# Genie-Kim/PintheMemory

Measured on AMD Instinct MI355X. Metric: train imgs/sec 768x768 bs=8 R50-DeepLabV3+ +mem, higher is better.
Workload: dtype f32

## Files before the change

### include/pinmem_hip.h

```cpp
#ifndef PINMEM_HIP_H
#define PINMEM_HIP_H
#include <stddef.h>
#include <stdint.h>

#ifdef __cplusplus
extern "C" {
#endif

typedef enum pm_status { PM_OK = 0, PM_EINVAL = -1, PM_EWORKSPACE = -2, PM_ELAUNCH = -3, PM_EUNSUPPORTED = -4 } pm_status;

typedef enum pm_dtype { PM_F32 = 0, PM_BF16 = 1 } pm_dtype;
#define PM_TF_ZERO_PAD64 1

typedef struct pm_tensor {
  void* ptr;
  int32_t n, h, w, c;
  int64_t pitch;
  int32_t dtype;
  int32_t flags;
} pm_tensor;

#define PM_ABI_VERSION 420

typedef struct pm_conv_params {
  int32_t struct_size;
  int32_t kh, kw, stride, pad, dil;
  int32_t prec;
  void* wino_v;
  int64_t wino_v_bytes;
  void* wxf;
  int64_t wxf_bytes;
  int32_t wxf_valid;
} pm_conv_params;

typedef struct pm_conv_epilogue {
  int64_t struct_size;
  const float* bias;
  const float* scale;
  const float* shift;
  const float* residual;
  int64_t residual_pitch;
  int32_t relu;
  float* bn_partials;
  int64_t bn_partials_bytes;
} pm_conv_epilogue;

const char* pm_last_error(void);
int pm_version(void);

size_t pm_conv_workspace(const pm_tensor* x, const pm_tensor* y, const pm_conv_params* p, int which );
size_t pm_conv_winograd_v_bytes(const pm_tensor* x, const pm_tensor* y, const pm_conv_params* p);
size_t pm_conv_wxf_bytes(const pm_tensor* x, const pm_tensor* y, const pm_conv_params* p);
size_t pm_conv_wxf_bytes_dgrad(const pm_tensor* dy, const pm_tensor* dx, const pm_conv_params* p);
typedef struct pm_wxf_job {
  const float* w;
  void* wxf;
  int64_t wxf_bytes;
  int32_t cout, kh, kw, cin;
  int32_t dgrad;
  int32_t reserved;
} pm_wxf_job;
int pm_conv_wxf_refresh_bf16(const pm_wxf_job* jobs, int n, void* stream);
int pm_conv_wxf_refresh_f32(const pm_wxf_job* jobs, int n, void* stream);
size_t pm_conv_bn_partials_bytes(const pm_tensor* x, const pm_tensor* y, const pm_conv_params* p);
int pm_conv_fwd(const pm_tensor* x, const float* w_krsc, const pm_tensor* y, const pm_conv_params* p,
                const pm_conv_epilogue* ep, void* ws, size_t ws_bytes, void* stream);
int pm_conv_bwd_data(const pm_tensor* dy, const float* w_krsc, const pm_tensor* dx, const pm_conv_params* p,
                     const pm_tensor* add, void* ws, size_t ws_bytes, void* stream);
int pm_conv_bwd_data_masked(const pm_tensor* dy, const float* w_krsc, const pm_tensor* dx, const pm_conv_params* p,
                            const pm_tensor* add, const uint8_t* add_mask, void* ws, size_t ws_bytes, void* stream);
int pm_conv_bwd_weight(const pm_tensor* x, const pm_tensor* dy, float* dw_krsc, float* dbias, const pm_conv_params* p,
                       void* ws, size_t ws_bytes, void* stream);

typedef struct pm_routing {
  int32_t struct_size;
  int32_t winograd;
  int32_t winograd_fused;
  int32_t conv16;
  int32_t conv16_wide;
  int32_t conv16_persistent;
  int32_t wgrad16;
  int32_t bf16_wgrad;
  int32_t split;
} pm_routing;
int pm_routing_get(pm_routing* out);
int pm_routing_set(const pm_routing* r);


int pm_set_winograd(int mode);
int pm_set_winograd_fused(int on);
int pm_set_conv16(int on);
int pm_set_bf16_wgrad(int on);
int pm_set_wgrad16(int on);
int pm_set_split(int on);

int pm_profile_enable(int on);
int pm_profile_dump(const char* csv_path);
int pm_profile_read(int mode, int bm, int bn, int km, int nst, double* total_ms, double* total_flops, int64_t* launches, int clear);
int pm_profile_read_prec(int mode, int bm, int bn, int km, int nst, int prec, double* total_ms, double* total_flops, int64_t* launches, int clear);
int pm_profile_read_bytes(int mode, int bm, int bn, int km, int nst, int prec, double* total_bytes);

size_t pm_bn_workspace(const pm_tensor* x);
int pm_bn_stats(const pm_tensor* x, float* moments, void* ws, size_t ws_bytes, void* stream);
int pm_bn_stats_finalize(const pm_tensor* x, float eps, float* mean, float* invstd, float* running_mean , float* running_var ,
                         float momentum, void* ws, size_t ws_bytes, void* stream);
int pm_bn_merge(const float* parts, int world, int c, float* moments, void* stream);
// ... 162 lines not shown
```

### pinthememory_amd/build.py

```python
import os
import subprocess
import sys

HERE = os.path.dirname(os.path.abspath(__file__))
CSRC = os.path.join(HERE, 'csrc')
LIB = os.path.join(HERE, 'libpinmem_hip.so')
SOURCES = ['misc.hip', 'bf16.hip', 'conv_igemm.hip', 'conv_split.hip', 'pwstream.hip', 'conv16.hip', 'conv16w.hip', 'wgrad16.hip', 'winograd.hip', 'bn.hip', 'pool_resize.hip', 'loss.hip', 'memory.hip', 'augment.hip', 'resample.hip']
FLAGS = ['--offload-arch=gfx950', '-O3', '-std=c++17', '-fPIC', '-ffp-contract=fast', '-Wall', '-Wno-unused-function']


STAMP = LIB + '.stamp'


def _fingerprint():
    import hashlib
    h = hashlib.sha256(' '.join(FLAGS).encode())
    for path in sorted(os.path.join(CSRC, f) for f in os.listdir(CSRC)) + [os.path.join(HERE, '..', 'include', 'pinmem_hip.h')]:
        h.update(os.path.basename(path).encode())
        with open(path, 'rb') as f:
            h.update(f.read())
    return h.hexdigest()


def _stale():
    if not (os.path.exists(LIB) and os.path.exists(STAMP)):
        return True
    with open(STAMP) as f:
        return f.read().strip() != _fingerprint()


# ... 47 lines not shown
```

### pinthememory_amd/csrc/conv_igemm.hip

```cpp
#include <stdlib.h>
#include <algorithm>
#include <type_traits>
#include <vector>

#include "pm_common.h"

#include "conv_igemm_kernel.h"

namespace {

template <int ZL, bool O16 = false>
__global__ __launch_bounds__(256) void splitk_reduce_vec_kernel(const float* __restrict__ ws, int ksplit, long slab, int M, int Nn,
                                                                float* __restrict__ C, long c_pitch, const float* bias,
                                                                const float* scale, const float* shift, const float* residual,
                                                                long res_pitch, int relu, const unsigned char* res_mask) {
  constexpr int GP = 256 / ZL;
  __shared__ float4 red[ZL > 1 ? ZL : 1][GP];
  const int gl = threadIdx.x % GP, zl = threadIdx.x / GP;
  const long groups = (long)M * Nn / 4;
  for (long g0 = (long)blockIdx.x * GP; g0 < groups; g0 += (long)gridDim.x * GP) {
    const long grp = g0 + gl;
    float4 v = make_float4(0.f, 0.f, 0.f, 0.f);
    if (grp < groups)
#pragma unroll 8
// ... 281 lines not shown
    if (k.prec == 2) return launch_prec<MODE, BM, BN, WM, WN, KM, 2>(k, grid, smem, st);
  }
  if constexpr (MODE == MODE_WGRAD && BN >= 64) {
    if (k.prec == 3) return launch_prec<MODE, BM, BN, WM, WN, KM, 3>(k, grid, smem, st);
    if (k.prec == 4) return launch_prec<MODE, BM, BN, WM, WN, KM, 4>(k, grid, smem, st);
  }
  if (k.prec != 0) launch_prec<MODE, BM, BN, WM, WN, KM, 1>(k, grid, smem, st);
  else launch_prec<MODE, BM, BN, WM, WN, KM, 0>(k, grid, smem, st);
}
template <int MODE, int BM, int BN, int WM, int WN>
void launch_one(const ConvK& k, dim3 grid, size_t smem, hipStream_t st) {
  if (k.kmode == K_SMALL) launch_inst<MODE, BM, BN, WM, WN, K_SMALL>(k, grid, smem, st);
  else if (k.kmode == K_FAST && MODE != MODE_WGRAD) launch_inst<MODE, BM, BN, WM, WN, (MODE != MODE_WGRAD ? K_FAST : K_MID)>(k, grid, smem, st);
  else launch_inst<MODE, BM, BN, WM, WN, K_MID>(k, grid, smem, st);
}

struct ProfRec {
  hipEvent_t a, b;
  int mode, bm, bn, km, prec, nst;
  int M, Nn, K, batch, ksplit;
  double flops;
  double bytes;
};
bool g_prof_on = false;
std::vector<ProfRec> g_prof;
struct ProfScope {
  ProfRec rec{};
  hipStream_t st;
  ProfScope(hipStream_t st_, int mode, int bm, int bn, int km, int prec, int nst, long M, long Nn, long K, int batch, int ksplit, double flops, double bytes = 0.0) : st(st_) {
    if (!g_prof_on) return;
    (void)hipEventCreate(&rec.a), (void)hipEventCreate(&rec.b);
    rec.mode = mode, rec.bm = bm, rec.bn = bn, rec.km = km, rec.prec = prec, rec.nst = nst, rec.M = (int)M, rec.Nn = (int)Nn, rec.K = (int)K, rec.batch = batch, rec.ksplit = ksplit;
    rec.flops = flops, rec.bytes = bytes;
    (void)hipEventRecord(rec.a, st);
  }
  void done() {
    if (!g_prof_on) return;
    (void)hipEventRecord(rec.b, st);
    g_prof.push_back(rec);
  }
};

template <class K>
void set_epilogue(K& k, const pm_conv_epilogue& e) {
  k.bias = e.bias, k.scale = e.scale, k.shift = e.shift, k.residual = e.residual, k.res_pitch = e.residual_pitch, k.relu = e.relu;
}
// ... 20 lines not shown
    k.batch_xcd = units >= 8 && (rem == 0 || ((rem == 1 || rem == 2 || rem == 4) && ntile % (8 / rem) == 0));
  }
  const int km = (MODE == MODE_WGRAD && k.kmode == K_FAST) ? K_MID : ((k.prec == 5 && MODE != MODE_WGRAD && k.kmode == K_FAST && k.kh * k.kw == 1 && k.stride == 1 && k.pad == 0 && !k.sub) ? K_PW : k.kmode);
  ProfScope prof(st, MODE, p.bm, p.bn, km, k.prec, lds_stages(MODE, k.kmode, p.bn, k.kper), k.M, k.Nn, k.K, batch, p.ksplit,
                 flops >= 0.0 ? flops : 2.0 * (double)k.M * (double)k.Nn * (double)k.K * batch,
                 (double)batch * ((double)k.a_bytes + (double)k.b_bytes + ((k.io16 && p.ksplit == 1) ? 2.0 : 4.0) * (double)k.M * (double)k.Nn * (double)p.ksplit));
  if constexpr (MODE != MODE_WGRAD) {
    if (pm_route.split && (k.prec == 0 || k.prec == 5) && !k.io16 && batch == 1 && p.ksplit == 1 && !k.stats && k.kh * k.kw == 1 && k.stride == 1 && k.pad == 0 && !k.sub) {
      pm_gemm_pw g;
      g.A = k.A, g.B = k.B, g.C = k.C, g.res_mask = k.res_mask;
      set_epilogue(g, pm_conv_epilogue{(int64_t)sizeof(pm_conv_epilogue), k.bias, k.scale, k.shift, k.residual, k.res_pitch, k.relu, nullptr, 0});
      g.a_pitch = MODE == MODE_FWD ? k.x_pitch : k.y_pitch, g.c_pitch = k.c_pitch;
      g.b_sn = MODE == MODE_FWD ? k.K : 1, g.b_sk = MODE == MODE_FWD ? 1 : k.Nn;
      g.M = k.M, g.Nn = k.Nn, g.K = k.K;
      if (pm_pwstream_ok(&g)) {
        prof.rec.bm = 32, prof.rec.bn = 64, prof.rec.km = 4, prof.rec.prec = 5, prof.rec.nst = 0;
        const int e = pm_pwstream_launch(&g, st);
        prof.done();
        return e;
      }
    }
  }
  constexpr bool akc = MODE != MODE_WGRAD, bkc = MODE == MODE_FWD;
  if (k.prec == 5) {
    if (int e = pm_conv_split_launch(MODE, p.bm, p.bn, k, grid.x, grid.y, grid.z, pm_conv_split_stage_bytes(MODE, p.bm, p.bn), st)) return e;
    prof.rec.nst = 1;
    prof.done();
    return pm_check_launch("conv_split");
  }
  const bool tr = MODE == MODE_WGRAD && (k.prec == 3 || k.prec == 4) && p.bn >= 64;
  auto smem = [&](int bm, int bn) {
    if (tr) return (size_t)2 * ((k.prec == 4 ? 2 : 1) * BK * (bm + 32) + (k.prec == 4 ? 2 : 1) * BK * (bn + 32)) * 2;
    return (size_t)2 * ((akc ? bm * LDK : BK * bm) + (bkc ? bn * LDK : BK * bn)) * sizeof(float);
  };
  if (p.bm == 64) {
    if (p.bn == 128) launch_one<MODE, 64, 128, 2, 2>(k, grid, smem(64, 128), st);
    else launch_one<MODE, 64, 64, 2, 2>(k, grid, smem(64, 64), st);
  } else if (p.bn == 128) {
    launch_one<MODE, 128, 128, 2, 2>(k, grid, smem(128, 128), st);
  } else if (p.bn == 64) {
    launch_one<MODE, 128, 64, 2, 2>(k, grid, smem(128, 64), st);
  } else {
    launch_one<MODE, 128, 32, 4, 1>(k, grid, smem(128, 32), st);
  }
  prof.done();
  return pm_check_launch("conv_igemm");
// ... 25 lines not shown
  }
  PM_REQUIRE(x->c % 4 == 0, PM_EUNSUPPORTED, "conv: Cin %% 4 != 0 unsupported (pad the input channels)");
  PM_REQUIRE((y->c % 4 == 0) || (p->kh * p->kw == 1), PM_EUNSUPPORTED, "conv: Cout %% 4 != 0 only for 1x1");
  PM_REQUIRE(x->pitch >= x->c && y->pitch >= y->c, PM_EINVAL, "conv: pitch < channels");
  PM_REQUIRE(pm_pixels(x) * x->pitch < (1ll << 29) && pm_pixels(y) * y->pitch < (1ll << 29) && (int64_t)y->c * x->c * p->kh * p->kw < (1ll << 29),
             PM_EUNSUPPORTED, "conv: tensor too large for 32-bit byte offsets (2 GiB per tensor)");
  return PM_OK;
}

void fill_geom(ConvK& k, const pm_tensor* x, const pm_tensor* y, const pm_conv_params* p) {
  k.N = x->n, k.H = x->h, k.W = x->w, k.Cin = x->c, k.x_pitch = x->pitch;
  k.Ho = y->h, k.Wo = y->w, k.Cout = y->c, k.y_pitch = y->pitch;
  k.kh = p->kh, k.kw = p->kw, k.stride = p->stride, k.pad = p->pad, k.dil = p->dil;
  k.sshift = p->stride == 2 ? 1 : 0;
  k.prec = p->prec != 0 ? 1 : 0;
  k.T_eff = p->kh * p->kw, k.tk_w = p->kw, k.ky0 = k.kx0 = 0, k.ksy = k.ksx = 1;
  k.sub = k.sub_cy = k.sub_cx = 0, k.Hc = x->h, k.Wc = x->w;
  k.bias = k.scale = k.shift = k.residual = nullptr;
  k.res_pitch = 0, k.res_mask = nullptr, k.relu = 0, k.stats = nullptr, k.io16 = 0;
  k.stage_ep = 1;
  k.spl_prio = 1;
  k.n_group = 8;
  k.batch_xcd = 0;
  k.a_bs = k.b_bs = k.c_bs = 0;
}

struct WinoPlan {
  bool use;
  pm_wino_geom g;
  int Kp, P;
  size_t v_bytes, m_bytes, u_bytes;
  Plan pl;
};
inline bool wino_wgrad_pays(int cin, int cout) { return (long)cin * cout >= 256 * 256; }
WinoPlan wino_plan(const pm_tensor* xin, int cout, const pm_conv_params* p, bool wgrad = false) {
  WinoPlan wp{};
  if (wgrad && !wino_wgrad_pays(xin->c, cout)) return wp;
  if (pm_route.winograd == 0 || p->kh != 3 || p->kw != 3 || p->stride != 1 || p->pad != p->dil || p->prec != 0) return wp;
  const int cin = xin->c;
  if (cin < 128 || cout < 128 || (cout & 3) || (cin & 3)) return wp;
  int m = 0;
  double best_ratio = 0.6;
  for (int cand = pm_route.winograd; cand >= 2; cand -= 2) {
    const pm_wino_geom g = pm_wino_make_geom(xin->n, xin->h, xin->w, p->dil, cand);
    const double cover = (double)(cand * g.TY * p->dil) * (double)(cand * g.TX * p->dil) / ((double)xin->h * xin->w);
    const double ratio = cover * (cand + 2) * (cand + 2) / (9.0 * cand * cand);
// ... 354 lines not shown
}

enum RouteKind {
  R_DIRECT,
  R_WINO,
  R_BF16,
  R_S2_NATIVE,
  R_S2_PARITY,
  R_WINO_WGRAD,
  R_BF16_WGRAD,
  R_DIRECT_WGRAD,
};
struct ConvRoute {
  RouteKind kind;
  Plan pl;
  WinoPlan wino;
  WinoWgradPlan wino_w;
  Bf16Plan b16;
  pm_conv_params pe;
  S2Native s2n;
  S2ParityPlan s2p;
  Bf16WgradPlan b16w;
  W16Plan w16;
  bool native16;
  size_t ws_bytes;
  size_t class_off, slab_off;
  size_t bias_off;
  size_t x32_off, dy32_off;
  size_t v_keep_bytes;
  size_t wxf_bytes;
  size_t bn_bytes;
};

ConvRoute route_conv(int which, const pm_tensor* x, const pm_tensor* y, const pm_conv_params* p) {
  ConvRoute r{};
  long M, Nn, K;
  gemm_dims(which, x, y, p, M, Nn, K);
  if (which == MODE_FWD) {
    if ((r.wino = wino_plan(x, y->c, p)).use) {
      r.kind = R_WINO, r.ws_bytes = wino_ws(r.wino), r.wxf_bytes = r.wino.u_bytes;
      r.v_keep_bytes = wino_wgrad_pays(x->c, y->c) ? r.wino.v_bytes : 0;
    } else if (p->prec == 2 && (r.b16 = bf16_plan(x, y, p)).use) {
      r.kind = R_BF16, r.pe = *p, r.ws_bytes = bf16_ws(r.b16), r.wxf_bytes = r.b16.wb_bytes;
    } else {
      r.kind = R_DIRECT, r.pl = make_plan(MODE_FWD, M, Nn, K, p->prec != 0), r.ws_bytes = pm_align_up(r.pl.ws_bytes, 256);
    }
    bool bn;
    if (pm_is_bf16(y)) bn = pm_vec8(y) && r.kind == R_BF16 && (r.b16.c16 ? (r.b16.k16.ksplit == 1 && !r.b16.k16.wide) : r.b16.pl.ksplit == 1);
    else if (pm_is_bf16(x) || (y->c & 3) || (y->pitch & 3) || !pm_aligned16(y->ptr)) bn = false;
    else bn = r.kind == R_BF16 ? r.b16.pl.ksplit == 1 : (r.kind == R_DIRECT && p->prec == 0 && r.pl.ksplit == 1 && r.pl.bn >= 64);
    r.bn_bytes = bn ? pm_align_up((size_t)pm_cdiv(pm_pixels(y), 32) * y->c * 2 * sizeof(float), 256) : 0;
  } else if (which == MODE_DGRAD) {
    if (p->stride == 2) {
      if ((r.s2n = s2_native_plan(y, x, p)).ok) {
        r.kind = R_S2_NATIVE, r.ws_bytes = r.s2n.total;
      } else {
        r.kind = R_S2_PARITY, r.s2p = s2_parity_plan(y, x, p);
        r.class_off = 0, r.slab_off = 4 * r.s2p.tmp_bytes;
        r.dy32_off = pm_align_up(r.slab_off + r.s2p.slab_bytes + 256, 256);
        r.ws_bytes = r.dy32_off + upcast_bytes(y);
      }
    } else if (dgrad_bf16_ok(p) && (r.pe = dgrad_as_fwd(p), r.b16 = bf16_plan(y, x, &r.pe)).use) {
      r.kind = R_BF16, r.ws_bytes = bf16_ws(r.b16), r.wxf_bytes = r.b16.wb_bytes;
    } else if ((r.wino = wino_plan(y, x->c, p)).use) {
      r.kind = R_WINO, r.ws_bytes = wino_ws(r.wino);
    } else {
      r.kind = R_DIRECT, r.pl = make_plan(MODE_DGRAD, M, Nn, K, p->prec != 0), r.ws_bytes = pm_align_up(r.pl.ws_bytes, 256);
    }
// ... 28 lines not shown
  const pm_tensor* dy = &dy32;
  float* tmp = (float*)((char*)ws + r.class_off);
  float* slab = (float*)((char*)ws + r.slab_off);
  for (int cls = 0; cls < 4; ++cls) {
    if (!r.s2p.valid[cls]) continue;
    const S2Class& c = r.s2p.c[cls];
    const Plan& pl = r.s2p.pl[cls];
    ConvK k;
    fill_geom(k, dx, dy, p);
    k.A = (const float*)dy->ptr, k.B = w;
    k.M = (int)c.M, k.Nn = dx->c, k.K = c.nky * c.nkx * dy->c;
    k.a_bytes = (unsigned)(pm_pixels(dy) * dy->pitch * 4), k.b_bytes = (unsigned)((long)dy->c * p->kh * p->kw * dx->c * 4);
    k.kmode = dy->c >= BK ? K_MID : K_SMALL;
    k.T_eff = c.nky * c.nkx, k.tk_w = c.nkx, k.ky0 = c.ky0, k.kx0 = c.kx0, k.ksy = c.ksy, k.ksx = c.ksx;
    k.sub = 1, k.sub_cy = c.cy, k.sub_cx = c.cx, k.Hc = c.Hc, k.Wc = c.Wc;
    float* out = (float*)((char*)tmp + cls * r.s2p.tmp_bytes);
    if (int e = run_gemm<MODE_DGRAD>(k, pl, slab, out, (long)dx->c, NO_EPILOGUE, st)) return e;
  }
  return s2_interleave(tmp, (long)(r.s2p.tmp_bytes / sizeof(float)), r.s2p.valid, dx, add, st, "dgrad_s2_interleave");
}

template <int MODE>
int conv_direct(const pm_tensor* x, const pm_tensor* y, const float* w, const pm_conv_params* p, const Plan& pl, const pm_conv_epilogue& e, void* ws, hipStream_t st,
                const unsigned char* res_mask = nullptr) {
  const pm_tensor *xin = MODE == MODE_FWD ? x : y, *out = MODE == MODE_FWD ? y : x;
  long M, Nn, K;
  gemm_dims(MODE, x, y, p, M, Nn, K);
  ConvK k;
  fill_geom(k, x, y, p);
  k.io16 = pm_is_bf16(out) ? 1 : 0;
  k.A = (const float*)xin->ptr, k.B = w;
  k.M = (int)M, k.Nn = (int)Nn, k.K = (int)K;
  k.a_bytes = (unsigned)(pm_pixels(xin) * xin->pitch * 4), k.b_bytes = (unsigned)((long)y->c * p->kh * p->kw * x->c * 4);
  k.kmode = (xin->c % BK == 0 && (MODE == MODE_FWD || p->stride == 1)) ? 0 : (xin->c >= BK ? 1 : 2);
  return run_gemm<MODE>(k, pl, (float*)ws, (float*)out->ptr, (long)out->pitch, e, st, -1.0, res_mask);
}

int conv_wgrad_direct(const pm_tensor* x, const pm_tensor* dy, float* dw, const pm_conv_params* p, const ConvRoute& r, void* ws, hipStream_t st) {
  long M, Nn, K;
  gemm_dims(MODE_WGRAD, x, dy, p, M, Nn, K);
  if (r.w16.use) {
    pm_wgrad16 w16 = r.w16.k;
    ProfScope prof(st, MODE_WGRAD, w16.bm, w16.bn, 2, 4, 3, M, Nn, K, 1, w16.ksplit, 2.0 * (double)M * (double)Nn * (double)K);
    return run_planned(w16.ksplit, M, Nn, (float*)ws, dw, Nn, NO_EPILOGUE, false, nullptr, st, [&](float* C, bool) {
      w16.C = C;
      const int e = pm_wgrad16_launch(&w16, st);
      prof.done();
      return e;
    });
  }
  ConvK k;
  fill_geom(k, x, dy, p);
  if (p->prec == 2) k.prec = 3;
  if (r.native16) {
    PM_REQUIRE(x->c % 8 == 0 && dy->c % 8 == 0 && r.pl.bn >= 64, PM_EUNSUPPORTED, "conv_bwd_weight(bf16): channels %% 8 != 0 or a tile narrower than 64");
    k.prec = 4;
  }
  const int esz = r.native16 ? 2 : 4;
  k.A = (const float*)dy->ptr, k.B = (const float*)x->ptr;
  k.M = (int)M, k.Nn = (int)Nn, k.K = (int)K;
  k.a_bytes = (unsigned)(pm_pixels(dy) * dy->pitch * esz), k.b_bytes = (unsigned)(pm_pixels(x) * x->pitch * esz), k.kmode = dy->w >= (r.native16 ? 2 * BK : BK) ? 1 : 2;
  return run_gemm<MODE_WGRAD>(k, r.pl, (float*)ws, dw, Nn, NO_EPILOGUE, st);
}

}

static pm_routing routing_from_env() {
  auto env = [](const char* name, int dflt) { const char* e = getenv(name); return e ? atoi(e) : dflt; };
  return pm_routing{
      (int32_t)sizeof(pm_routing),
      4,
      env("PM_WINO_FUSED", 0),
      env("PM_CONV16", 1),
      env("PM_C16W", 1),
      env("PM_C16P", 1),
      env("PM_WGRAD16", 1),
      0,
      env("PM_SPLIT", 1),
  };
}
const pm_routing pm_route_defaults = routing_from_env();
pm_routing pm_route = pm_route_defaults;
extern "C" int pm_routing_get(pm_routing* out) {
  PM_REQUIRE(out && out->struct_size == (int32_t)sizeof(pm_routing), PM_EINVAL, "pm_routing_get: struct_size %d != %zu (library ABI %d)", out ? out->struct_size : -1,
             sizeof(pm_routing), PM_ABI_VERSION);
  *out = pm_route;
  return PM_OK;
}
extern "C" int pm_routing_set(const pm_routing* r) {
  PM_REQUIRE(r && r->struct_size == (int32_t)sizeof(pm_routing), PM_EINVAL, "pm_routing_set: struct_size %d != %zu (library ABI %d)", r ? r->struct_size : -1, sizeof(pm_routing),
             PM_ABI_VERSION);
  PM_REQUIRE(r->winograd == 0 || r->winograd == 2 || r->winograd == 4, PM_EINVAL, "pm_routing_set: winograd %d (0, 2 or 4)", r->winograd);
  PM_REQUIRE(r->conv16 >= 0 && r->conv16 <= 2 && r->conv16_wide >= 0 && r->conv16_wide <= 3, PM_EINVAL, "pm_routing_set: conv16 %d / conv16_wide %d", r->conv16, r->conv16_wide);
  pm_route = *r;
  return PM_OK;
}
extern "C" int pm_set_winograd(int mode) {
  PM_REQUIRE(mode == 0 || mode == 2 || mode == 4, PM_EINVAL, "pm_set_winograd: mode %d (0 off, 2 F(2x2,3x3), 4 prefer F(4x4,3x3))", mode);
  pm_route.winograd = mode;
  return PM_OK;
}
extern "C" int pm_set_conv16(int on) {
  PM_REQUIRE(on >= 0 && on <= 8, PM_EINVAL, "pm_set_conv16: %d (0 register-staged, 1 per shape, 2 LDS-DMA everywhere / narrow tiles only, 3 LDS-DMA everywhere / wide tiles "
             "wherever the shape allows, 4 per shape without the wide kernel, 5 / 6 = 1 (the streaming 1x1 kernel left the library in round 6), 7 as 3 with the 256 x 256 tile, "
             "8 as 3 with one block per tile instead of the persistent ring)", on);
  pm_route.conv16 = (on == 3 || on == 7 || on == 8) ? 2 : ((on == 4 || on == 5 || on == 6) ? 1 : on);
  pm_route.conv16_wide = (on == 3 || on == 8) ? 2 : (on == 7 ? 3 : ((on == 2 || on == 4) ? 0 : pm_route_defaults.conv16_wide));
  pm_route.conv16_persistent = on == 8 ? 0 : (on == 3 ? 1 : pm_route_defaults.conv16_persistent);
  return PM_OK;
}
extern "C" int pm_set_winograd_fused(int on) {
  pm_route.winograd_fused = on != 0;
  return PM_OK;
}
extern "C" int pm_set_wgrad16(int on) {
  pm_route.wgrad16 = on != 0;
// ... 60 lines not shown
  }
  fclose(f);
  return PM_OK;
}

extern "C" size_t pm_conv_workspace(const pm_tensor* x, const pm_tensor* y, const pm_conv_params* p0, int which) {
  const pm_conv_params tp = tier_params(p0, x, y);
  return route_conv(which, x, y, &tp).ws_bytes;
}
extern "C" size_t pm_conv_winograd_v_bytes(const pm_tensor* x, const pm_tensor* y, const pm_conv_params* p0) {
  if (!x || !y || !p0) return 0;
  const pm_conv_params tp = tier_params(p0, x, y);
  return route_conv(MODE_FWD, x, y, &tp).v_keep_bytes;
}
extern "C" size_t pm_conv_wxf_bytes(const pm_tensor* x, const pm_tensor* y, const pm_conv_params* p0) {
  if (!x || !y || !p0) return 0;
  const pm_conv_params tp = tier_params(p0, x, y);
  return route_conv(MODE_FWD, x, y, &tp).wxf_bytes;
}
extern "C" size_t pm_conv_wxf_bytes_dgrad(const pm_tensor* dy, const pm_tensor* dx, const pm_conv_params* p0) {
  if (!dy || !dx || !p0) return 0;
  const pm_conv_params tp = tier_params(p0, dy, dx);
  return route_conv(MODE_DGRAD, dx, dy, &tp).wxf_bytes;
}
extern "C" size_t pm_conv_bn_partials_bytes(const pm_tensor* x, const pm_tensor* y, const pm_conv_params* p0) {
  if (!x || !y || !p0 || check_common(x, y, p0) != PM_OK) return 0;
  const pm_conv_params tp = tier_params(p0, x, y);
  return route_conv(MODE_FWD, x, y, &tp).bn_bytes;
}

extern "C" int pm_conv_wxf_refresh_f32(const pm_wxf_job* jobs, int n, void* stream) {
  PM_REQUIRE(n >= 0 && (jobs || n == 0), PM_EINVAL, "conv_wxf_refresh_f32: bad job table");
  std::vector<const float*> w(n);
  std::vector<float*> U(n);
  std::vector<int> cout(n), cin(n), kp(n), m(n);
  for (int i = 0; i < n; ++i) {
    const pm_wxf_job& q = jobs[i];
    PM_REQUIRE(q.w && q.wxf && q.cout > 0 && q.cin > 0 && q.kh == 3 && q.kw == 3 && q.dgrad == 0, PM_EINVAL,
               "conv_wxf_refresh_f32: job %d: forward transforms of 3x3 filters only", i);
    PM_REQUIRE(pm_aligned16(q.wxf), PM_EINVAL, "conv_wxf_refresh_f32: job %d: buffer must be 16-byte aligned", i);
    const int Kp = (q.cin + BK - 1) / BK * BK;
    const size_t u4 = pm_align_up((size_t)36 * q.cout * Kp * sizeof(float), 256), u2 = pm_align_up((size_t)16 * q.cout * Kp * sizeof(float), 256);
    PM_REQUIRE((size_t)q.wxf_bytes == u4 || (size_t)q.wxf_bytes == u2, PM_EINVAL, "conv_wxf_refresh_f32: job %d: %ld bytes is neither the F(4x4) nor the F(2x2) transform of %d x %d",
               i, (long)q.wxf_bytes, q.cout, q.cin);
    w[i] = q.w, U[i] = (float*)q.wxf, cout[i] = q.cout, cin[i] = q.cin, kp[i] = Kp, m[i] = (size_t)q.wxf_bytes == u4 ? 4 : 2;
  }
// ... 11 lines not shown
  PM_REQUIRE(w && pm_aligned16(w), PM_EINVAL, "conv_fwd: weight null or unaligned");
  pm_conv_epilogue e0 = {(int64_t)sizeof(pm_conv_epilogue), nullptr, nullptr, nullptr, nullptr, 0, 0};
  if (ep) e0 = *ep;
  PM_REQUIRE((e0.scale == nullptr) == (e0.shift == nullptr), PM_EINVAL, "conv_fwd: scale and shift go together");
  const ConvRoute r = route_conv(MODE_FWD, x, y, p);
  if (e0.bn_partials) {
    PM_REQUIRE(!e0.relu && !e0.residual, PM_EINVAL, "conv_fwd: bn_partials are the statistics of the convolution output (no residual / ReLU)");
    PM_REQUIRE(r.bn_bytes != 0 && (size_t)e0.bn_partials_bytes >= r.bn_bytes, PM_EINVAL, "conv_fwd: this call cannot emit bn_partials (ask pm_conv_bn_partials_bytes): %zu needed", r.bn_bytes);
  }
  PM_REQUIRE(ws_bytes >= r.ws_bytes && (ws || r.ws_bytes == 0), PM_EWORKSPACE, "conv_fwd: workspace %zu < %zu", ws_bytes, r.ws_bytes);
  hipStream_t st = (hipStream_t)stream;
  switch (r.kind) {
    case R_WINO: {
      float* keep = (p->wino_v && (size_t)p->wino_v_bytes >= r.wino.v_bytes) ? (float*)p->wino_v : nullptr;
      float* uext = (p->wxf && (size_t)p->wxf_bytes >= r.wino.u_bytes) ? (float*)p->wxf : nullptr;
      return wino_conv(x, w, y->c, x->c, false, y, r.wino, e0, ws, st, keep, uext, p->wxf_valid != 0);
    }
    case R_BF16: {
      char* wext = (p->wxf && (size_t)p->wxf_bytes >= r.b16.wb_bytes) ? (char*)p->wxf : nullptr;
      return conv_bf16(x, w, y->c, x->c, false, y, &r.pe, r.b16, e0, ws, st, wext, p->wxf_valid != 0);
    }
    default:
      PM_REQUIRE(pm_is_f32(x), PM_EUNSUPPORTED, "conv_fwd: a bf16 input needs at least 32 channels (got %d)", x->c);
      return conv_direct<MODE_FWD>(x, y, w, p, r.pl, e0, ws, st);
  }
}

extern "C" int pm_conv_bwd_data(const pm_tensor* dy, const float* w, const pm_tensor* dx, const pm_conv_params* p0, const pm_tensor* add,
                                void* ws, size_t ws_bytes, void* stream) {
  return pm_conv_bwd_data_masked(dy, w, dx, p0, add, nullptr, ws, ws_bytes, stream);
}

extern "C" int pm_conv_bwd_data_masked(const pm_tensor* dy, const float* w, const pm_tensor* dx, const pm_conv_params* p0, const pm_tensor* add,
                                       const uint8_t* add_mask, void* ws, size_t ws_bytes, void* stream) {
  if (int e = check_common(dx, dy, p0)) return e;
  const pm_conv_params tp = tier_params(p0, dy, dx);
  const pm_conv_params* p = &tp;
  PM_REQUIRE(!add || (add->ptr && pm_same_shape(add, dx) && add->dtype == dx->dtype), PM_EINVAL, "conv_bwd_data: `add` must match dx (shape and dtype)");
  PM_REQUIRE(!add || !pm_is_bf16(add) || pm_vec8(add), PM_EINVAL, "conv_bwd_data: bf16 `add` must be 16B aligned with pitch %% 8 == 0");
  PM_REQUIRE(w && pm_aligned16(w), PM_EINVAL, "conv_bwd_data: weight null or unaligned");
  const ConvRoute r = route_conv(MODE_DGRAD, dx, dy, p);
  PM_REQUIRE(ws_bytes >= r.ws_bytes && (ws || r.ws_bytes == 0), PM_EWORKSPACE, "conv_bwd_data: workspace %zu < %zu", ws_bytes, r.ws_bytes);
  if (add_mask) {
    PM_REQUIRE(add && pm_is_f32(add) && pm_is_f32(dy) && pm_vec4(add) && pm_vec4(dx), PM_EINVAL, "conv_bwd_data: a masked `add` is an fp32 tensor with 16-byte rows and c %% 4 == 0");
    PM_REQUIRE(r.kind == R_DIRECT, PM_EUNSUPPORTED,
               "conv_bwd_data: a masked `add` is served by the fp32 implicit-GEMM route only (this call routes to %s)",
               r.kind == R_WINO ? "Winograd" : (r.kind == R_BF16 ? "the bf16 kernels" : "the stride-2 class kernels"));
// ... 55 lines not shown
```

### pinthememory_amd/csrc/conv_igemm_parts.h

```cpp
#pragma once
#include <stdint.h>
#include <type_traits>

#include "pm_common.h"

typedef float f32x16 __attribute__((ext_vector_type(16)));
typedef __bf16 bf16x8 __attribute__((ext_vector_type(8)));

struct ConvK {
  const float* A;
  const float* B;
  float* C;
  int N, H, W, Cin;
  int Ho, Wo, Cout;
  long x_pitch, y_pitch;
  int kh, kw, stride, pad, dil, sshift;
  int M, Nn, K;
  int ksplit;
  int kper;
  long c_pitch;
  long c_split;
  long a_bs, b_bs, c_bs;
  int tiles_m, tiles_n;
  unsigned a_bytes, b_bytes;
  int kmode;
  int prec;
  int T_eff, tk_w, ky0, kx0, ksy, ksx;
  int sub, sub_cy, sub_cx, Hc, Wc;
  const float* bias;
  const float* scale;
  const float* shift;
  const float* residual;
  long res_pitch;
  const unsigned char* res_mask;
  int relu;
  float* stats;
  int io16;
  int stage_ep;
  int n_group;
  int batch_xcd;
  int spl_prio;
};

namespace {

enum { MODE_FWD = 0, MODE_DGRAD = 1, MODE_WGRAD = 2 };
constexpr int BK = 32;
constexpr int LDK = 36;
constexpr int LD5 = 52;

typedef float v4f __attribute__((ext_vector_type(4)));
constexpr int OOB = 0x7fffffff;

__device__ __forceinline__ v4f bload(__amdgpu_buffer_rsrc_t r, unsigned off) {
  return __builtin_bit_cast(v4f, __builtin_amdgcn_raw_buffer_load_b128(r, (int)off, 0, 0));
}

__device__ __forceinline__ uint2 pack4(const v4f& v) {
  typedef __bf16 bf16x4 __attribute__((ext_vector_type(4)));
  bf16x4 o;
  o[0] = (__bf16)v.x, o[1] = (__bf16)v.y, o[2] = (__bf16)v.z, o[3] = (__bf16)v.w;
  return __builtin_bit_cast(uint2, o);
}
__device__ __forceinline__ void split4(const v4f& v, uint2& hi, uint2& mid, uint2& lo) {
  const unsigned u0 = __float_as_uint(v.x), u1 = __float_as_uint(v.y), u2 = __float_as_uint(v.z), u3 = __float_as_uint(v.w);
// ... 228 lines not shown
```

### pinthememory_amd/hip/lib.py

```python
import ctypes
import os
from ctypes import POINTER, byref, c_char_p, c_float, c_int, c_int32, c_int64, c_size_t, c_void_p

import torch

_HERE = os.path.dirname(os.path.dirname(os.path.abspath(__file__)))
LIB_PATH = os.environ.get('PM_LIB') or os.path.join(_HERE, 'libpinmem_hip.so')


class PmTensor(ctypes.Structure):
    _fields_ = [('ptr', c_void_p), ('n', c_int32), ('h', c_int32), ('w', c_int32), ('c', c_int32), ('pitch', c_int64), ('dtype', c_int32), ('flags', c_int32)]


PM_F32, PM_BF16 = 0, 1
PM_TF_ZERO_PAD64 = 1


class PmSgdEntry(ctypes.Structure):
    _fields_ = [('param', c_void_p), ('grad', c_void_p), ('momentum_buffer', c_void_p), ('numel', c_int64)]


class PmWxfJob(ctypes.Structure):
    _fields_ = [('w', c_void_p), ('wxf', c_void_p), ('wxf_bytes', c_int64), ('cout', c_int32), ('kh', c_int32), ('kw', c_int32), ('cin', c_int32),
                ('dgrad', c_int32), ('reserved', c_int32)]


class PmConvParams(ctypes.Structure):
    _fields_ = [('struct_size', c_int32), ('kh', c_int32), ('kw', c_int32), ('stride', c_int32), ('pad', c_int32), ('dil', c_int32), ('prec', c_int32),
                ('wino_v', c_void_p), ('wino_v_bytes', c_int64),
                ('wxf', c_void_p), ('wxf_bytes', c_int64), ('wxf_valid', c_int32)]


class PmRouting(ctypes.Structure):
    _fields_ = [('struct_size', c_int32), ('winograd', c_int32), ('winograd_fused', c_int32), ('conv16', c_int32), ('conv16_wide', c_int32),
                ('conv16_persistent', c_int32), ('wgrad16', c_int32), ('bf16_wgrad', c_int32), ('split', c_int32)]


class PmAugImage(ctypes.Structure):
    _fields_ = [('order', ctypes.c_uint8 * 4), ('enabled', ctypes.c_uint8), ('flip', ctypes.c_uint8), ('hue_shift', ctypes.c_uint8), ('reserved', ctypes.c_uint8),
                ('brightness', c_float), ('contrast', c_float), ('saturation', c_float), ('radius', c_int32), ('w', ctypes.c_double * 6)]


class PmGeoImage(ctypes.Structure):
    _fields_ = [('h_in', c_int32), ('w_in', c_int32), ('h', c_int32), ('w', c_int32), ('pad_h', c_int32), ('pad_w', c_int32), ('y1', c_int32), ('x1', c_int32)]


RESAMPLE_MAX_TAPS = 24
RESAMPLE_REC = RESAMPLE_MAX_TAPS + 2


class PmConvEpilogue(ctypes.Structure):
    _fields_ = [('struct_size', c_int64), ('bias', c_void_p), ('scale', c_void_p), ('shift', c_void_p), ('residual', c_void_p),
                ('residual_pitch', c_int64), ('relu', c_int32), ('bn_partials', c_void_p), ('bn_partials_bytes', c_int64)]


def conv_params(kh, kw, stride, pad, dil, prec=0):
    return PmConvParams(ctypes.sizeof(PmConvParams), kh, kw, stride, pad, dil, prec)


def conv_epilogue(*fields):
    return PmConvEpilogue(ctypes.sizeof(PmConvEpilogue), *fields)


ABI_VERSION = 420


class PinmemError(RuntimeError):
    pass


_T, _P, _E = POINTER(PmTensor), POINTER(PmConvParams), POINTER(PmConvEpilogue)
_vp, _sz, _i, _f, _i64 = c_void_p, c_size_t, c_int, c_float, c_int64

SIGNATURES = {
    'pm_last_error': (c_char_p, []),
    'pm_version': (c_int, []),
    'pm_conv_winograd_v_bytes': (_sz, [_T, _T, _P]),
    'pm_conv_wxf_bytes': (_sz, [_T, _T, _P]),
    'pm_conv_wxf_bytes_dgrad': (_sz, [_T, _T, _P]),
    'pm_conv_wxf_refresh_bf16': (_i, [_vp, _i, _vp]),
    'pm_conv_wxf_refresh_f32': (_i, [_vp, _i, _vp]),
    'pm_conv_workspace': (_sz, [_T, _T, _P, _i]),
    'pm_conv_fwd': (_i, [_T, _vp, _T, _P, _E, _vp, _sz, _vp]),
    'pm_conv_bwd_data': (_i, [_T, _vp, _T, _P, _T, _vp, _sz, _vp]),
    'pm_conv_bwd_data_masked': (_i, [_T, _vp, _T, _P, _T, _vp, _vp, _sz, _vp]),
    'pm_conv_bwd_weight': (_i, [_T, _T, _vp, _vp, _P, _vp, _sz, _vp]),
    'pm_set_winograd': (_i, [_i]),
# ... 65 lines not shown
    'pm_label_class_weights_workspace': (_sz, [_i]),
    'pm_label_class_weights': (_i, [_vp, _i, _i, _i, _i, ctypes.c_double, _i, _i, _vp, _vp, _sz, _vp]),
    'pm_upsample_eval_workspace': (_sz, [_T, _i, _i]),
    'pm_upsample_eval': (_i, [_T, _f, _vp, _i, _i, _vp, _vp, _i, _vp, _vp, _sz, _vp]),
    'pm_mem_read_fwd': (_i, [_T, _vp, _i, _vp, _T, _vp, _vp, _vp]),
    'pm_mem_read_fwd_pq_workspace': (_sz, [_i64, _i]),
    'pm_mem_read_fwd_pq': (_i, [_T, _vp, _i, _vp, _vp, _T, _vp, _vp, _vp, _vp, _sz, _vp]),
    'pm_mem_colsoftmax_workspace': (_sz, [_i64, _i]),
    'pm_mem_colsoftmax': (_i, [_vp, _vp, _i64, _i, _vp, _vp, _sz, _vp]),
    'pm_mem_read_bwd_workspace': (_sz, [_i64, _i, _i]),
    'pm_mem_read_bwd': (_i, [_T, _vp, _i, _vp, _T, _vp, _T, _vp, _vp, _sz, _vp]),
    'pm_mem_write_accum_workspace': (_sz, [_T, _i]),
    'pm_mem_write_accum': (_i, [_T, _vp, _i, _i, _i, _i, _vp, _vp, _sz, _vp]),
    'pm_mem_write_accum_bwd': (_i, [_T, _vp, _i, _i, _i, _i, _vp, _T, _vp]),
    'pm_mem_write_update': (_i, [_vp, _vp, _i, _i, _f, _vp, _vp, _vp]),
    'pm_mem_write_update_bwd': (_i, [_vp, _vp, _i, _i, _f, _vp, _vp, _vp, _vp]),
    'pm_sgd_momentum': (_i, [_vp, _vp, _vp, _i64, _f, _f, _f, _i, _vp]),
    'pm_set_bf16_wgrad': (_i, [_i]),
    'pm_set_wgrad16': (_i, [_i]),
    'pm_set_split': (_i, [_i]),
    'pm_routing_get': (_i, [POINTER(PmRouting)]),
    'pm_routing_set': (_i, [POINTER(PmRouting)]),
    'pm_conv_bn_partials_bytes': (_sz, [_T, _T, POINTER(PmConvParams)]),
    'pm_bn_partials_finalize': (_i, [_vp, _i64, _i, _f, _vp, _vp, _vp, _vp, _f, _vp, _vp]),
    'pm_sgd_momentum_multi': (_i, [_vp, _i, _f, _f, _f, _vp]),
    'pm_sgd_momentum_multi_dev': (_i, [_vp, _i, _f, _vp, _f, _f, _vp]),
    'pm_cast': (_i, [_T, _T, _vp]),
}

_lib = None


def load():
    global _lib
    if _lib is not None:
        return _lib
    if not os.environ.get('PM_LIB'):
        from .. import build as _build
        _build.build()
    lib = ctypes.CDLL(LIB_PATH)
    for name, (res, args) in SIGNATURES.items():
        fn = getattr(lib, name)
        fn.restype, fn.argtypes = res, args
    if lib.pm_version() != ABI_VERSION:
        raise PinmemError('%s reports ABI %d, this binding is written against %d (include/pinmem_hip.h)' % (LIB_PATH, lib.pm_version(), ABI_VERSION))
    _lib = lib
# ... 82 lines not shown
```

Baseline: 156.8.

## Add dedicated persistent LDS-halo kernel for the 7x7 stride-2 stem convolution

Adds a specialized forward kernel for the ResNet stem conv (7x7, stride 2, 4-channel padded input, 64 outputs). It loads the whole weight matrix once per block and stages an input halo patch in LDS, in a parity-split layout so stride-2 taps read contiguously. It runs persistently over patches, prefetching the next halo while the MFMA bf16x3 split-precision products run. This replaces the generic split-precision implicit GEMM path, which re-gathers overlapping input windows from global memory. The kernel is enabled by default for large inputs and uses most of the LDS, which limits occupancy.

```diff
diff --git a/include/pinmem_hip.h b/include/pinmem_hip.h
--- a/include/pinmem_hip.h
+++ b/include/pinmem_hip.h
@@ -20,7 +20,7 @@
   int32_t flags;
 } pm_tensor;
 
-#define PM_ABI_VERSION 420
+#define PM_ABI_VERSION 421
 
 typedef struct pm_conv_params {
   int32_t struct_size;
@@ -63,6 +63,7 @@
 int pm_conv_wxf_refresh_bf16(const pm_wxf_job* jobs, int n, void* stream);
 int pm_conv_wxf_refresh_f32(const pm_wxf_job* jobs, int n, void* stream);
 size_t pm_conv_bn_partials_bytes(const pm_tensor* x, const pm_tensor* y, const pm_conv_params* p);
+size_t pm_conv_fwd_stem_lds_bytes(const pm_tensor* x, const pm_tensor* y, const pm_conv_params* p);
 int pm_conv_fwd(const pm_tensor* x, const float* w_krsc, const pm_tensor* y, const pm_conv_params* p,
                 const pm_conv_epilogue* ep, void* ws, size_t ws_bytes, void* stream);
 int pm_conv_bwd_data(const pm_tensor* dy, const float* w_krsc, const pm_tensor* dx, const pm_conv_params* p,
@@ -82,6 +83,7 @@
   int32_t wgrad16;
   int32_t bf16_wgrad;
   int32_t split;
+  int32_t stem;
 } pm_routing;
 int pm_routing_get(pm_routing* out);
 int pm_routing_set(const pm_routing* r);
diff --git a/pinthememory_amd/build.py b/pinthememory_amd/build.py
--- a/pinthememory_amd/build.py
+++ b/pinthememory_amd/build.py
@@ -5,7 +5,7 @@
 HERE = os.path.dirname(os.path.abspath(__file__))
 CSRC = os.path.join(HERE, 'csrc')
 LIB = os.path.join(HERE, 'libpinmem_hip.so')
-SOURCES = ['misc.hip', 'bf16.hip', 'conv_igemm.hip', 'conv_split.hip', 'pwstream.hip', 'conv16.hip', 'conv16w.hip', 'wgrad16.hip', 'winograd.hip', 'bn.hip', 'pool_resize.hip', 'loss.hip', 'memory.hip', 'augment.hip', 'resample.hip']
+SOURCES = ['misc.hip', 'bf16.hip', 'conv_igemm.hip', 'conv_split.hip', 'stem.hip', 'pwstream.hip', 'conv16.hip', 'conv16w.hip', 'wgrad16.hip', 'winograd.hip', 'bn.hip', 'pool_resize.hip', 'loss.hip', 'memory.hip', 'augment.hip', 'resample.hip']
 FLAGS = ['--offload-arch=gfx950', '-O3', '-std=c++17', '-fPIC', '-ffp-contract=fast', '-Wall', '-Wno-unused-function']
 
 
diff --git a/pinthememory_amd/csrc/conv_igemm.hip b/pinthememory_amd/csrc/conv_igemm.hip
--- a/pinthememory_amd/csrc/conv_igemm.hip
+++ b/pinthememory_amd/csrc/conv_igemm.hip
@@ -327,6 +327,7 @@
   double flops;
   double bytes;
 };
+constexpr int STEM_BM = 256, STEM_KM = 5;
 bool g_prof_on = false;
 std::vector<ProfRec> g_prof;
 struct ProfScope {
@@ -393,6 +394,15 @@
     }
   }
   constexpr bool akc = MODE != MODE_WGRAD, bkc = MODE == MODE_FWD;
+  if constexpr (MODE == MODE_FWD) {
+    if (k.stem && k.prec == 5 && batch == 1 && p.ksplit == 1 && !k.stats && !k.io16 && ((k.c_pitch | (k.residual ? k.res_pitch : 0)) & 3) == 0 &&
+        ((reinterpret_cast<uintptr_t>(k.C) | reinterpret_cast<uintptr_t>(k.residual)) & 15) == 0) {
+      prof.rec.bm = STEM_BM, prof.rec.bn = 64, prof.rec.km = STEM_KM, prof.rec.nst = 1;
+      const int e = pm_conv_stem_launch(k, st);
+      prof.done();
+      return e;
+    }
+  }
   if (k.prec == 5) {
     if (int e = pm_conv_split_launch(MODE, p.bm, p.bn, k, grid.x, grid.y, grid.z, pm_conv_split_stage_bytes(MODE, p.bm, p.bn), st)) return e;
     prof.rec.nst = 1;
@@ -464,6 +474,7 @@
   k.spl_prio = 1;
   k.n_group = 8;
   k.batch_xcd = 0;
+  k.stem = 0;
   k.a_bs = k.b_bs = k.c_bs = 0;
 }
 
@@ -864,6 +875,7 @@
   S2ParityPlan s2p;
   Bf16WgradPlan b16w;
   W16Plan w16;
+  bool stem;
   bool native16;
   size_t ws_bytes;
   size_t class_off, slab_off;
@@ -873,6 +885,13 @@
   size_t wxf_bytes;
   size_t bn_bytes;
 };
+
+constexpr long STEM_MIN_PIXELS = 256l * 256 * 4;
+bool stem_takes(const pm_tensor* x, const pm_tensor* y, const pm_conv_params* p, long M, const Plan& pl) {
+  if (pm_route.stem == 0 || !pm_route.split || p->prec != 0 || !pm_is_f32(x) || !pm_is_f32(y)) return false;
+  if (p->kh != 7 || p->kw != 7 || p->stride != 2 || p->pad != 3 || p->dil != 1 || x->c != 4 || y->c != 64 || pl.ksplit != 1) return false;
+  return pm_route.stem == 2 || M >= STEM_MIN_PIXELS;
+}
 
 ConvRoute route_conv(int which, const pm_tensor* x, const pm_tensor* y, const pm_conv_params* p) {
   ConvRoute r{};
@@ -886,6 +905,7 @@
       r.kind = R_BF16, r.pe = *p, r.ws_bytes = bf16_ws(r.b16), r.wxf_bytes = r.b16.wb_bytes;
     } else {
       r.kind = R_DIRECT, r.pl = make_plan(MODE_FWD, M, Nn, K, p->prec != 0), r.ws_bytes = pm_align_up(r.pl.ws_bytes, 256);
+      r.stem = stem_takes(x, y, p, M, r.pl);
     }
     bool bn;
     if (pm_is_bf16(y)) bn = pm_vec8(y) && r.kind == R_BF16 && (r.b16.c16 ? (r.b16.k16.ksplit == 1 && !r.b16.k16.wide) : r.b16.pl.ksplit == 1);
@@ -960,7 +980,7 @@
 
 template <int MODE>
 int conv_direct(const pm_tensor* x, const pm_tensor* y, const float* w, const pm_conv_params* p, const Plan& pl, const pm_conv_epilogue& e, void* ws, hipStream_t st,
-                const unsigned char* res_mask = nullptr) {
+                const unsigned char* res_mask = nullptr, bool stem = false) {
   const pm_tensor *xin = MODE == MODE_FWD ? x : y, *out = MODE == MODE_FWD ? y : x;
   long M, Nn, K;
   gemm_dims(MODE, x, y, p, M, Nn, K);
@@ -971,6 +991,7 @@
   k.M = (int)M, k.Nn = (int)Nn, k.K = (int)K;
   k.a_bytes = (unsigned)(pm_pixels(xin) * xin->pitch * 4), k.b_bytes = (unsigned)((long)y->c * p->kh * p->kw * x->c * 4);
   k.kmode = (xin->c % BK == 0 && (MODE == MODE_FWD || p->stride == 1)) ? 0 : (xin->c >= BK ? 1 : 2);
+  k.stem = stem ? 1 : 0;
   return run_gemm<MODE>(k, pl, (float*)ws, (float*)out->ptr, (long)out->pitch, e, st, -1.0, res_mask);
 }
 
@@ -1015,6 +1036,7 @@
       env("PM_WGRAD16", 1),
       0,
       env("PM_SPLIT", 1),
+      1,
   };
 }
 const pm_routing pm_route_defaults = routing_from_env();
@@ -1030,6 +1052,7 @@
              PM_ABI_VERSION);
   PM_REQUIRE(r->winograd == 0 || r->winograd == 2 || r->winograd == 4, PM_EINVAL, "pm_routing_set: winograd %d (0, 2 or 4)", r->winograd);
   PM_REQUIRE(r->conv16 >= 0 && r->conv16 <= 2 && r->conv16_wide >= 0 && r->conv16_wide <= 3, PM_EINVAL, "pm_routing_set: conv16 %d / conv16_wide %d", r->conv16, r->conv16_wide);
+  PM_REQUIRE(r->stem >= 0 && r->stem <= 2, PM_EINVAL, "pm_routing_set: stem %d (0 never, 1 by rule, 2 whenever the geometry fits)", r->stem);
   pm_route = *r;
   return PM_OK;
 }
@@ -1136,6 +1159,11 @@
   if (!dy || !dx || !p0) return 0;
   const pm_conv_params tp = tier_params(p0, dy, dx);
   return route_conv(MODE_DGRAD, dx, dy, &tp).wxf_bytes;
+}
+extern "C" size_t pm_conv_fwd_stem_lds_bytes(const pm_tensor* x, const pm_tensor* y, const pm_conv_params* p0) {
+  if (!x || !y || !p0 || check_common(x, y, p0) != PM_OK) return 0;
+  const pm_conv_params tp = tier_params(p0, x, y);
+  return route_conv(MODE_FWD, x, y, &tp).stem ? pm_conv_stem_lds() : 0;
 }
 extern "C" size_t pm_conv_bn_partials_bytes(const pm_tensor* x, const pm_tensor* y, const pm_conv_params* p0) {
   if (!x || !y || !p0 || check_common(x, y, p0) != PM_OK) return 0;
@@ -1193,7 +1221,7 @@
     }
     default:
       PM_REQUIRE(pm_is_f32(x), PM_EUNSUPPORTED, "conv_fwd: a bf16 input needs at least 32 channels (got %d)", x->c);
-      return conv_direct<MODE_FWD>(x, y, w, p, r.pl, e0, ws, st);
+      return conv_direct<MODE_FWD>(x, y, w, p, r.pl, e0, ws, st, nullptr, r.stem);
   }
 }
 
diff --git a/pinthememory_amd/csrc/conv_igemm_parts.h b/pinthememory_amd/csrc/conv_igemm_parts.h
--- a/pinthememory_amd/csrc/conv_igemm_parts.h
+++ b/pinthememory_amd/csrc/conv_igemm_parts.h
@@ -40,7 +40,11 @@
   int n_group;
   int batch_xcd;
   int spl_prio;
-};
+  int stem;
+};
+
+int pm_conv_stem_launch(const ConvK& k, hipStream_t st);
+size_t pm_conv_stem_lds();
 
 namespace {
 
diff --git a/pinthememory_amd/csrc/stem.hip b/pinthememory_amd/csrc/stem.hip
--- /dev/null
+++ b/pinthememory_amd/csrc/stem.hip
@@ -0,0 +1,174 @@
+#include <algorithm>
+#include <type_traits>
+
+#include "conv_igemm_parts.h"
+
+namespace {
+
+constexpr int ST_PH = 8, ST_PW = 32;
+constexpr int ST_HH = 2 * ST_PH + 5, ST_HW = 2 * ST_PW + 5;
+constexpr int ST_HALO = ST_HH * ST_HW;
+constexpr int ST_THREADS = 512, ST_HPT = (ST_HALO + ST_THREADS - 1) / ST_THREADS;
+constexpr int ST_ODD = (ST_HW + 1) / 2 * 8;
+constexpr int ST_AROW = ST_HW * 8 + 8, ST_APLANE = ST_HH * ST_AROW;
+constexpr int ST_TAPS = 49, ST_KPAD = 224, ST_K = 196;
+constexpr int ST_BROW = ST_KPAD * 2 + 16, ST_BPLANE = 64 * ST_BROW;
+constexpr int ST_B_BYTES = 3 * ST_BPLANE, ST_A_BYTES = 3 * ST_APLANE;
+constexpr int ST_EP_BYTES = 8 * 32 * (32 + 4) * 4;
+constexpr int ST_LDS_BYTES = ST_B_BYTES + ST_A_BYTES + ST_EP_BYTES;
+static_assert(ST_LDS_BYTES <= 160 * 1024 && ST_B_BYTES % 16 == 0 && (ST_B_BYTES + ST_A_BYTES) % 16 == 0, "stem kernel LDS plan");
+static_assert(ST_HW / 2 + 1 <= ST_ODD / 8 && ST_ODD + (ST_HW / 2) * 8 <= ST_AROW, "halo row layout");
+
+constexpr int st_tap(int t) { return (t / 7) * ST_AROW + ((t % 7) & 1) * ST_ODD + ((t % 7) >> 1) * 8; }
+
+template <int EPF>
+__global__ __launch_bounds__(ST_THREADS) __attribute__((amdgpu_waves_per_eu(2, 2))) void conv_stem_fwd_kernel(const ConvK a) {
+  extern __shared__ __align__(16) float smem[];
+  char* Bs = reinterpret_cast<char*>(smem);
+  char* As = Bs + ST_B_BYTES;
+  float* Es = reinterpret_cast<float*>(As + ST_A_BYTES);
+
+  const int t = threadIdx.x;
+  const int lane = t & 63, wave = t >> 6;
+  const int wm = wave >> 1, wn = wave & 1;
+  const int half = lane >> 5, l31 = lane & 31;
+
+  const __amdgpu_buffer_rsrc_t rA = __builtin_amdgcn_make_buffer_rsrc(const_cast<float*>(a.A), 0, (int)a.a_bytes, 0x00020000);
+  const __amdgpu_buffer_rsrc_t rB = __builtin_amdgcn_make_buffer_rsrc(const_cast<float*>(a.B), 0, (int)a.b_bytes, 0x00020000);
+  const int xp4 = (int)a.x_pitch * 4;
+
+  for (int e = t; e < 64 * (ST_KPAD / 4); e += ST_THREADS) {
+    const int row = e / (ST_KPAD / 4), q = e - row * (ST_KPAD / 4);
+    const v4f v = bload(rB, q < ST_TAPS ? (row * ST_K + q * 4) * 4 : OOB);
+    uint2 s[3];
+    split4(v, s[0], s[1], s[2]);
+#pragma unroll
+    for (int p = 0; p < 3; ++p) *reinterpret_cast<uint2*>(Bs + p * ST_BPLANE + row * ST_BROW + q * 8) = s[p];
+  }
+
+  int hy[ST_HPT], hx[ST_HPT], hdst[ST_HPT];
+#pragma unroll
+  for (int j = 0; j < ST_HPT; ++j) {
+    const int e = t + ST_THREADS * j;
+    hy[j] = e / ST_HW, hx[j] = e - hy[j] * ST_HW;
+    hdst[j] = e < ST_HALO ? hy[j] * ST_AROW + (hx[j] & 1) * ST_ODD + (hx[j] >> 1) * 8 : -1;
+  }
+  const int npatch = a.N * a.tiles_m * a.tiles_n;
+  v4f ra[ST_HPT];
+  auto load_halo = [&](int p) {
+    const int img = p / (a.tiles_m * a.tiles_n), rem = p - img * (a.tiles_m * a.tiles_n);
+    const int ty = rem / a.tiles_n, tx = rem - ty * a.tiles_n;
+    const int iy0 = 2 * ty * ST_PH - 3, ix0 = 2 * tx * ST_PW - 3;
+#pragma unroll
+    for (int j = 0; j < ST_HPT; ++j) {
+      const int iy = iy0 + hy[j], ix = ix0 + hx[j];
+      const bool ok = (p < npatch) & (hdst[j] >= 0) & ((unsigned)iy < (unsigned)a.H) & ((unsigned)ix < (unsigned)a.W);
+      ra[j] = bload(rA, ok ? ((img * a.H + iy) * a.W + ix) * xp4 : OOB);
+    }
+  };
+  auto write_halo = [&]() {
+#pragma unroll
+    for (int j = 0; j < ST_HPT; ++j) {
+      uint2 s[3];
+      split4(ra[j], s[0], s[1], s[2]);
+      if (hdst[j] >= 0) {
+#pragma unroll
+        for (int p = 0; p < 3; ++p) *reinterpret_cast<uint2*>(As + p * ST_APLANE + hdst[j]) = s[p];
+      }
+    }
+  };
+
+  const char* afrag = As + wm * 2 * ST_AROW + l31 * 8;
+  const char* bfrag = Bs + (wn * 32 + l31) * ST_BROW + half * 16;
+  const bool plain = !(a.bias || a.scale || a.residual || a.relu);
+  const bool aff = EPF == 3 ? !plain && (a.bias || a.scale) : EPF >= 1, res = EPF == 3 ? !plain && a.residual : false, relu = EPF == 3 ? !plain && a.relu : EPF == 2;
+  ConvK ep = a;
+
+  int p = blockIdx.x;
+  load_halo(p);
+  write_halo();
+  __syncthreads();
+  for (; p < npatch; p += gridDim.x) {
+    load_halo(p + gridDim.x);
+    f32x16 acc[2][1][1];
+#pragma unroll
+    for (int i = 0; i < 2; ++i)
+#pragma unroll
+      for (int q = 0; q < 16; ++q) acc[i][0][0][q] = 0.f;
+
+    bf16x8 fa[2][3][2], fb[2][3];
+    auto read_frags = [&](auto gc, bf16x8 (&xa)[3][2], bf16x8 (&xb)[3]) {
+      constexpr int g = decltype(gc)::value, t0 = 4 * g, t1 = 4 * g + 2;
+      constexpr bool any = t0 < ST_TAPS;
+      const int o0 = half ? (t1 < ST_TAPS ? st_tap(t1) : 0) : (any ? st_tap(t0) : 0);
+      const int o1 = half ? (t1 + 1 < ST_TAPS ? st_tap(t1 + 1) : 0) : (t0 + 1 < ST_TAPS ? st_tap(t0 + 1) : 0);
+      const bool z0 = half ? !(t1 < ST_TAPS) : !any, z1 = half ? !(t1 + 1 < ST_TAPS) : !(t0 + 1 < ST_TAPS);
+#pragma unroll
+      for (int pl = 0; pl < 3; ++pl) {
+#pragma unroll
+        for (int i = 0; i < 2; ++i) {
+          uint2 lo = make_uint2(0u, 0u), hi = make_uint2(0u, 0u);
+          if constexpr (any) {
+            lo = *reinterpret_cast<const uint2*>(afrag + pl * ST_APLANE + i * 8 * ST_AROW + o0);
+            hi = *reinterpret_cast<const uint2*>(afrag + pl * ST_APLANE + i * 8 * ST_AROW + o1);
+            if constexpr (t1 + 1 >= ST_TAPS) {
+              lo = z0 ? make_uint2(0u, 0u) : lo;
+              hi = z1 ? make_uint2(0u, 0u) : hi;
+            }
+          }
+          xa[pl][i] = __builtin_bit_cast(bf16x8, make_uint4(lo.x, lo.y, hi.x, hi.y));
+        }
+        xb[pl] = __builtin_bit_cast(bf16x8, *reinterpret_cast<const v4f*>(bfrag + pl * ST_BPLANE + g * 32));
+      }
+    };
+    auto k_group = [&](auto gc) {
+      constexpr int g = decltype(gc)::value, cur = g & 1;
+      if constexpr (g + 1 < ST_KPAD / 16) read_frags(std::integral_constant<int, g + 1>{}, fa[cur ^ 1], fb[cur ^ 1]);
+      __builtin_amdgcn_sched_barrier(0);
+#define PM_ST_PROD(PA, PB) \
+  _Pragma("unroll") for (int i = 0; i < 2; ++i) acc[i][0][0] = __builtin_amdgcn_mfma_f32_32x32x16_bf16(fa[cur][PA][i], fb[cur][PB], acc[i][0][0], 0, 0, 0);
+      PM_ST_PROD(2, 0) PM_ST_PROD(0, 2) PM_ST_PROD(1, 1) PM_ST_PROD(1, 0) PM_ST_PROD(0, 1) PM_ST_PROD(0, 0)
+#undef PM_ST_PROD
+      __builtin_amdgcn_sched_barrier(0);
+    };
+    read_frags(std::integral_constant<int, 0>{}, fa[0], fb[0]);
+#define PM_ST_G(G) k_group(std::integral_constant<int, G>{});
+    PM_ST_G(0) PM_ST_G(1) PM_ST_G(2) PM_ST_G(3) PM_ST_G(4) PM_ST_G(5) PM_ST_G(6) PM_ST_G(7) PM_ST_G(8) PM_ST_G(9) PM_ST_G(10) PM_ST_G(11) PM_ST_G(12) PM_ST_G(13)
+#undef PM_ST_G
+    static_assert(ST_KPAD / 16 == 14, "the K groups are written out");
+
+    __syncthreads();
+    write_halo();
+    const int img = p / (a.tiles_m * a.tiles_n), rem = p - img * (a.tiles_m * a.tiles_n);
+    const int ty = rem / a.tiles_n, tx = rem - ty * a.tiles_n;
+#pragma unroll
+    for (int i = 0; i < 2; ++i) {
+      const int oy = ty * ST_PH + wm + 4 * i, ox0 = tx * ST_PW;
+      const int m0 = (img * a.Ho + oy) * a.Wo + ox0;
+      ep.M = oy < a.Ho ? m0 + min(ST_PW, a.Wo - ox0) : 0;
+      igemm_epilogue_staged<float, false, false, 128, 64, 1, 2>(ep, a.C, a.residual, Es, acc[i], m0, 0, 0, wn, wave, lane, l31, half, aff, res, relu);
+    }
+  }
+}
+
+template <int EPF>
+void stem_launch(const ConvK& k, hipStream_t st) {
+  static pm_lds_optin optin;
+  const int cus = optin(reinterpret_cast<const void*>(conv_stem_fwd_kernel<EPF>), 160 * 1024);
+  const long npatch = (long)k.N * k.tiles_m * k.tiles_n;
+  hipLaunchKernelGGL(conv_stem_fwd_kernel<EPF>, dim3((unsigned)std::min<long>(npatch, cus)), dim3(ST_THREADS), ST_LDS_BYTES, st, k);
+}
+
+}
+
+size_t pm_conv_stem_lds() { return ST_LDS_BYTES; }
+
+int pm_conv_stem_launch(const ConvK& k0, hipStream_t st) {
+  ConvK k = k0;
+  k.tiles_m = pm_cdiv(k.Ho, ST_PH), k.tiles_n = pm_cdiv(k.Wo, ST_PW);
+  const bool plain = !(k.bias || k.scale || k.residual || k.relu), aff = k.bias || k.scale;
+  if (plain) stem_launch<0>(k, st);
+  else if (aff && !k.residual) k.relu ? stem_launch<2>(k, st) : stem_launch<1>(k, st);
+  else stem_launch<3>(k, st);
+  return pm_check_launch("conv_stem");
+}
diff --git a/pinthememory_amd/hip/lib.py b/pinthememory_amd/hip/lib.py
--- a/pinthememory_amd/hip/lib.py
+++ b/pinthememory_amd/hip/lib.py
@@ -33,7 +33,7 @@
 
 class PmRouting(ctypes.Structure):
     _fields_ = [('struct_size', c_int32), ('winograd', c_int32), ('winograd_fused', c_int32), ('conv16', c_int32), ('conv16_wide', c_int32),
-                ('conv16_persistent', c_int32), ('wgrad16', c_int32), ('bf16_wgrad', c_int32), ('split', c_int32)]
+                ('conv16_persistent', c_int32), ('wgrad16', c_int32), ('bf16_wgrad', c_int32), ('split', c_int32), ('stem', c_int32)]
 
 
 class PmAugImage(ctypes.Structure):
@@ -62,7 +62,7 @@
     return PmConvEpilogue(ctypes.sizeof(PmConvEpilogue), *fields)
 
 
-ABI_VERSION = 420
+ABI_VERSION = 421
 
 
 class PinmemError(RuntimeError):
@@ -174,6 +174,7 @@
     'pm_routing_get': (_i, [POINTER(PmRouting)]),
     'pm_routing_set': (_i, [POINTER(PmRouting)]),
     'pm_conv_bn_partials_bytes': (_sz, [_T, _T, POINTER(PmConvParams)]),
+    'pm_conv_fwd_stem_lds_bytes': (_sz, [_T, _T, POINTER(PmConvParams)]),
     'pm_bn_partials_finalize': (_i, [_vp, _i64, _i, _f, _vp, _vp, _vp, _vp, _f, _vp, _vp]),
     'pm_sgd_momentum_multi': (_i, [_vp, _i, _f, _f, _f, _vp]),
     'pm_sgd_momentum_multi_dev': (_i, [_vp, _i, _f, _vp, _f, _f, _vp]),
```

Result: no change. 157.3, median of 6 (+0.4%).
